# JuliaGeometry/Raycore.jl

Measured on AMD Instinct MI355X. Metric: Mrays/s closest_hit (1M-tri TLAS), higher is better.
Workload: dtype f32; 1 GPU; C3: TLAS of 256 rotated/scaled instances of one 4096-triangle BLAS (1 048 576 triangles), 4194304 pinhole primary rays per GPU per step, closest_hit; triangles=1048576, kernel=auto (phased persistent, top level in LDS), parallelism=replicas x1 (rays sharded, no collective)

## Files before the change

raycore.jl_amd/csrc/rc_build.hip:

```cpp
#include <hipcub/hipcub.hpp>
#include <rocprim/rocprim.hpp>

#include <algorithm>
#include <cmath>
#include <cstring>

#include "rc_internal.h"

namespace {

constexpr int kBlock = 256;
inline unsigned grid_for(uint64_t n) { return (unsigned)((n + kBlock - 1) / kBlock); }

__host__ __device__ inline uint32_t enc_f32(float f) {
    uint32_t u = __builtin_bit_cast(uint32_t, f);
    return (u & 0x80000000u) ? ~u : (u | 0x80000000u);
}
__host__ __device__ inline float dec_f32(uint32_t e) {
    uint32_t u = (e & 0x80000000u) ? (e & 0x7FFFFFFFu) : ~e;
    return __builtin_bit_cast(float, u);
}

__device__ inline void block_reduce_bounds(float3_ mn, float3_ mx, uint32_t* partials) {
    uint32_t e[6] = {enc_f32(mn.x), enc_f32(mn.y), enc_f32(mn.z), enc_f32(mx.x), enc_f32(mx.y), enc_f32(mx.z)};
// ... 744 lines not shown
    emit_tree(s, out.nodes.p, n, s->range_tmp);
    hipLaunchKernelGGL(k_blas_leaves, dim3(grid_for(n)), dim3(kBlock), 0, s->stream, out.nodes.p, out.prims.p, n);
    run_refit(s, out.nodes.p, out.prims.p, n, 0, s->range_tmp);
    rc_timing_scene_end(s, s->stream);
    RcNode root;
    RC_HIP(hipMemcpyAsync(&root, out.nodes.p, sizeof(RcNode), hipMemcpyDeviceToHost, s->stream));
    RC_HIP(hipStreamSynchronize(s->stream));
    RC_HIP(hipGetLastError());
    host_root_aabb(root, false, out.root_min, out.root_max);
}

static void pack_tlas(rc_scene* s) {
    const uint32_t n = (s->n_tlas_nodes + 1) / 2;
    if (s->tlas_top_k) hipLaunchKernelGGL(k_pack_nodes_remap, dim3(grid_for(s->n_tlas_nodes)), dim3(kBlock), 0, s->stream, s->tlas_nodes.p, s->flat_nodes.p + s->n_flat_nodes, s->n_tlas_nodes, n, s->tlas_remap.p, false);
    else hipLaunchKernelGGL(k_pack_nodes, dim3(grid_for(s->n_tlas_nodes)), dim3(kBlock), 0, s->stream, s->tlas_nodes.p, s->flat_nodes.p + s->n_flat_nodes, s->n_tlas_nodes, 0u);
}

void rc_build_tlas(rc_scene* s) {
    const uint32_t n = (uint32_t)s->instances.size();
    const uint32_t nb = (uint32_t)s->blas.size();
    s->descs.resize(nb);
    uint32_t tn = 0, tp = 0;
    for (uint32_t i = 0; i < nb; ++i) {
        s->descs[i].nodes_offset = tn; s->descs[i].primitives_offset = tp;
        memcpy(s->descs[i].root_min, s->blas[i].root_min, 12); memcpy(s->descs[i].root_max, s->blas[i].root_max, 12);
        tn += s->blas[i].n_nodes; tp += s->blas[i].n_prims;
    }
    s->n_flat_nodes = tn; s->n_flat_prims = tp;
    s->flat_attrs_valid = false;
    s->vf_order_valid = false;
    s->flat_nodes.reserve((size_t)tn + 2 * (size_t)n + 1);
    s->flat_prims.reserve(tp ? tp : 1);
    s->d_descs.reserve(nb ? nb : 1);
    s->blas_top_k = 0;
    s->tlas_top_k = 0;
    s->blas_top_k32 = 0;
    s->tlas_top_k32 = 0;
    s->small_trees = n <= rc::kStack16MaxLeaves;
    for (uint32_t i = 0; i < nb; ++i) s->small_trees = s->small_trees && s->blas[i].n_prims <= rc::kStack16MaxLeaves;
    const bool full_lds = n > 0 && 2 * n - 1 <= (uint32_t)rc::kTlasLdsNodes;
    const bool small_enough = (uint64_t)tn + 2ull * n < (1ull << 26);
    uint32_t blas_room = 0, blas_room32 = 0;
    auto split = [&](uint32_t P, uint32_t& tk, uint32_t& bk) {
        const uint32_t t_int = n - 1, b_int = (nb == 1 && s->blas[0].n_prims >= 2) ? s->blas[0].n_prims - 1 : 0;
        tk = t_int < P ? t_int : P; bk = b_int < P ? b_int : P;
        if (tk + bk > P) {
            const uint32_t half = P / 2;
            if (tk <= half) bk = P - tk; else if (bk <= half) tk = P - bk; else { tk = P - half; bk = half; }
        }
    };
    if (s->opt.blas_top && n > 0 && small_enough) {
        if (full_lds) {
            blas_room32 = (uint32_t)rc::kLdsPlaneNodes - (n - 1);
            blas_room = s->small_trees ? (uint32_t)rc::kLdsPlaneNodes16 - (n - 1) : blas_room32;
        } else {
            uint32_t tk, bk, tk32, bk32;
            split((uint32_t)rc::kPartialPlaneNodes, tk32, bk32);
            if (s->small_trees) split((uint32_t)rc::kPartialPlaneNodes16, tk, bk); else { tk = tk32; bk = bk32; }
            if (tk32 > tk) tk32 = tk;
            if (bk32 > bk) bk32 = bk;
            s->tlas_top_k = tk; s->tlas_top_k32 = tk32;
            blas_room = bk; blas_room32 = bk32;
        }
    }
    if (nb == 1 && blas_room > 0 && s->blas[0].n_prims >= 2) {
        const uint32_t n_leaves = s->blas[0].n_prims, n_int = n_leaves - 1, room = blas_room;
        s->blas_top_k = n_int < room ? n_int : room;
        s->blas_top_k32 = s->blas_top_k < blas_room32 ? s->blas_top_k : blas_room32;
        s->top_remap.reserve(n_int);
        hipLaunchKernelGGL(k_iota1, dim3(grid_for(n_int)), dim3(kBlock), 0, s->stream, s->top_remap.p, n_int);
        hipLaunchKernelGGL(k_top_remap, dim3(1), dim3(kTopBlock), 0, s->stream, s->blas[0].nodes.p, n_leaves, s->blas_top_k, s->top_remap.p);
    }
    for (uint32_t i = 0; i < nb; ++i) {
        if (s->blas_top_k) hipLaunchKernelGGL(k_pack_nodes_remap, dim3(grid_for(s->blas[i].n_nodes)), dim3(kBlock), 0, s->stream, s->blas[i].nodes.p, s->flat_nodes.p + s->descs[i].nodes_offset, s->blas[i].n_nodes, s->blas[i].n_prims, s->top_remap.p, true);
        else hipLaunchKernelGGL(k_pack_nodes, dim3(grid_for(s->blas[i].n_nodes)), dim3(kBlock), 0, s->stream, s->blas[i].nodes.p, s->flat_nodes.p + s->descs[i].nodes_offset, s->blas[i].n_nodes, s->blas[i].n_prims);
        RC_HIP(hipMemcpyAsync(s->flat_prims.p + s->descs[i].primitives_offset, s->blas[i].prims.p, sizeof(RcPrim) * s->blas[i].n_prims, hipMemcpyDeviceToDevice, s->stream));
    }
    if (nb) RC_HIP(hipMemcpyAsync(s->d_descs.p, s->descs.data(), sizeof(RcBlasDesc) * nb, hipMemcpyHostToDevice, s->stream));
    s->blas_nprims.resize(nb);
    for (uint32_t i = 0; i < nb; ++i) s->blas_nprims[i] = s->blas[i].n_prims;
    s->d_blas_nprims.reserve(nb ? nb : 1);
    if (nb) RC_HIP(hipMemcpyAsync(s->d_blas_nprims.p, s->blas_nprims.data(), sizeof(uint32_t) * nb, hipMemcpyHostToDevice, s->stream));
    s->blas_cull_bits.reserve(nb ? nb : 1);
    RC_HIP(hipMemsetAsync(s->blas_cull_bits.p, 0, sizeof(uint32_t) * (nb ? nb : 1), s->stream));
    if (nb && tp) hipLaunchKernelGGL(k_cull_radius, dim3(grid_for(tp)), dim3(kBlock), 0, s->stream, s->flat_prims.p, tp, s->d_descs.p, nb, s->blas_cull_bits.p);
    s->n_static_instances = n;
    if (n == 0) {
        s->n_tlas_nodes = 0;
        for (int k = 0; k < 3; ++k) { s->root_min[k] = INFINITY; s->root_max[k] = -INFINITY; }
        RC_HIP(hipStreamSynchronize(s->stream));
        return;
    }
    reserve_build_scratch(s, n);
    s->d_instances.reserve(n); s->inst_recs.reserve(n); s->inst_cull.reserve(2 * (size_t)n); s->aabb_tmp.reserve(6 * (size_t)n);
    s->tlas_nodes.reserve(2 * (size_t)n - 1);
    s->n_tlas_nodes = 2 * n - 1;
    RC_HIP(hipMemcpyAsync(s->d_instances.p, s->instances.data(), sizeof(RcInstanceDesc) * n, hipMemcpyHostToDevice, s->stream));
    hipLaunchKernelGGL(k_inst_recs, dim3(grid_for(n)), dim3(kBlock), 0, s->stream, s->d_instances.p, s->d_descs.p, s->d_blas_nprims.p, n, s->inst_recs.p,
                       (const uint32_t*)s->blas_cull_bits.p, s->inst_cull.p);
    s->bounds_partials.reserve((size_t)grid_for(n) * 6);
    hipLaunchKernelGGL(k_instance_aabbs, dim3(grid_for(n)), dim3(kBlock), 0, s->stream, s->d_instances.p, s->d_descs.p, n, s->aabb_tmp.p, s->bounds_partials.p);
    hipLaunchKernelGGL(k_reduce_partials, dim3(1), dim3(384), 0, s->stream, s->bounds_partials.p, grid_for(n), s->scene_enc.p);
    hipLaunchKernelGGL(k_tlas_morton, dim3(grid_for(n)), dim3(kBlock), 0, s->stream, s->d_instances.p, s->d_descs.p, n, s->scene_enc.p, s->keys_a.p, s->vals_a.p);
    sort_pairs(s, n);
    emit_tree(s, s->tlas_nodes.p, n, s->tlas_ranges);
    hipLaunchKernelGGL(k_tlas_leaves, dim3(grid_for(n)), dim3(kBlock), 0, s->stream, s->tlas_nodes.p, s->vals_b.p, s->d_instances.p, s->d_descs.p, n);
    run_refit(s, s->tlas_nodes.p, nullptr, n, 1, s->tlas_ranges);
// ... 35 lines not shown
```

raycore.jl_amd/csrc/rc_internal.h:

```cpp
#pragma once
#include <hip/hip_runtime.h>

#include <condition_variable>
#include <map>
#include <memory>
#include <mutex>
#include <set>
#include <stdexcept>
#include <string>
#include <vector>

#include "rc_device.h"

struct RcError : std::runtime_error {
    int code;
    RcError(int c, const std::string& m) : std::runtime_error(m), code(c) {}
};

#define RC_HIP(expr)                                                                                      \
    do {                                                                                                  \
        hipError_t _e = (expr);                                                                           \
        if (_e != hipSuccess)                                                                             \
            throw RcError(4, std::string(#expr) + " failed: " + hipGetErrorString(_e) + " (" __FILE__ ":" + \
                                 std::to_string(__LINE__) + ")");                                         \
// ... 37 lines not shown
    }
};

struct RcEvent {
    hipEvent_t e = nullptr;
    bool recorded = false, owned = false;
    RcEvent() = default;
    RcEvent(const RcEvent&) = delete;
    RcEvent& operator=(const RcEvent&) = delete;
    RcEvent(RcEvent&& o) noexcept : e(o.e), recorded(o.recorded), owned(o.owned) { o.e = nullptr; o.recorded = o.owned = false; }
    RcEvent& operator=(RcEvent&& o) noexcept { if (this != &o) { drop(); e = o.e; recorded = o.recorded; owned = o.owned; o.e = nullptr; o.recorded = o.owned = false; } return *this; }
    ~RcEvent() { drop(); }
    void drop() { if (e && owned) (void)hipEventDestroy(e); e = nullptr; recorded = owned = false; }
    void record(hipStream_t st) {
        if (e && !owned) drop();
        if (!e) { if (hipEventCreateWithFlags(&e, hipEventDisableTiming) != hipSuccess) { (void)hipGetLastError(); e = nullptr; return; } owned = true; }
        if (hipEventRecord(e, st) == hipSuccess) recorded = true; else (void)hipGetLastError();
    }
    void follow(hipEvent_t closing) { drop(); e = closing; recorded = closing != nullptr; }
    bool idle() const {
        if (!recorded) return true;
        const hipError_t q = hipEventQuery(e);
        if (q != hipSuccess) (void)hipGetLastError();
        return q == hipSuccess;
    }
    void wait() const { if (recorded && hipEventSynchronize(e) != hipSuccess) (void)hipGetLastError(); }
};

struct Blas {
    DevBuf<RcNode> nodes;
    DevBuf<RcPrim> prims;
    uint32_t n_prims = 0;
    uint32_t n_nodes = 0;
    float root_min[3] = {0, 0, 0}, root_max[3] = {0, 0, 0};
    DevBuf<float> m_normals, m_uvs;
    DevBuf<uint32_t> m_indices, src_face;
    bool has_attrs = false, has_uvs = false;
    uint32_t n_mesh_verts = 0, n_mesh_faces = 0;
    DevBuf<RcNode4> nodes4;
    uint32_t n_nodes4 = 0;
    uint32_t root_word4 = 1;
};

struct HandleRange {
    uint32_t first = 0, count = 0;
};

namespace rc {
constexpr int kTlasLdsNodes = 511;
constexpr int kTlasLdsInst = 256;
constexpr int kLdsPlaneNodes = 310;
constexpr int kPartialPlaneNodes = 585;
#ifndef RC_LDS_PLANES16
#define RC_LDS_PLANES16 748
#endif
constexpr int kLdsPlaneNodes16 = RC_LDS_PLANES16;
constexpr int kPartialPlaneNodes16 = 1023;
constexpr uint32_t kStack16MaxLeaves = 32767;
}

struct TraceOptions {
    int64_t kernel = -1;
    int64_t blocks_per_cu = 0;
    int64_t lds_stack = 24;
    int64_t pool = 0;
    int64_t refill = 20;
    int64_t sched_thr = 36;
    int64_t stats = 0;
    int64_t onesweep_min = 1000000;
    int64_t stack16 = 1;
    int64_t blas_top = 1;
    int64_t host_pipeline = 1;
    int64_t taper = 12;
    int64_t entry_cull = 1;
    int64_t cost_order = 1;
    int64_t cost_thr = 64;
    int64_t claim_shards = 16;
    int64_t vf_first_touch = 1;
    int64_t vf_chunk_bytes = 192 << 20;
    int64_t timeline_ptr = 0;
};

struct TimingRef {
    int slot = -2;
    uint64_t seq = 0;
    float fixed_ms = 0.f;
};

struct RcCaptureRelaxed {
    hipStreamCaptureMode mode = hipStreamCaptureModeRelaxed;
    RcCaptureRelaxed() { (void)hipThreadExchangeStreamCaptureMode(&mode); }
    ~RcCaptureRelaxed() { (void)hipThreadExchangeStreamCaptureMode(&mode); }
    RcCaptureRelaxed(const RcCaptureRelaxed&) = delete;
    RcCaptureRelaxed& operator=(const RcCaptureRelaxed&) = delete;
};

struct CallCtx {
    hipStream_t stream = nullptr;
    bool own_stream = false;
    bool busy = false;
    DevBuf<RcRay> rays;
    DevBuf<RcHit> hits;
};

struct rc_scene {
    int device = 0;
    int n_cus = 0;
    uint64_t uid = 0;
    hipStream_t stream = nullptr;
// ... 203 lines not shown
```

raycore.jl_amd/csrc/rc_traverse.hip:

```cpp
#include <algorithm>
#include <cstdlib>

#include <hip/hip_ext.h>
#include <hipcub/hipcub.hpp>

#include "rc_traverse_core.h"

namespace {

using namespace rc;

template <bool ANY, int LDS_N, int MINW>
__global__ __launch_bounds__(kBlock, MINW) void k_trace_simple(TraceArgs a) {
    __shared__ uint32_t lds_stack[LDS_N * kBlock];
    const uint32_t gtid = blockIdx.x * kBlock + threadIdx.x;
    LaneStackT<LDS_N> st(lds_stack + threadIdx.x, a.v.overflow + gtid, a.v.total_threads, a.v.status);
    for (uint64_t i = gtid; i < a.n_rays; i += a.v.total_threads) {
        RayState s;
        init_ray(s, load_ray(a.rays, i), ANY, st, a.v.tlas_off);
        if (a.v.n_tlas_nodes != 0)
            while (step<ANY>(s, a.v, st)) {}
        write_hit(s, a.v, a.hits, i);
    }
}
// ... 19 lines not shown
    s.node = RC_INVALID_NODE;
    unsigned long long st_steps = 0, st_lanes = 0, st_maxsp = 0;
    for (;;) {
        unsigned long long idle_mask = __ballot(!active);
        int n_idle = __popcll(idle_mask);
        const bool can_refill = !(exhausted && pool_next == pool_end);
        if (n_idle == 64 && !can_refill) break;
        if (can_refill && n_idle >= a.refill) {
            for (;;) {
                idle_mask = __ballot(!active);
                n_idle = __popcll(idle_mask);
                if (n_idle == 0) break;
                if (pool_next == pool_end) {
                    if (exhausted) break;
                    if (!rc_claim_chunk(a.claim, nullptr, (blockIdx.x * kBlock + threadIdx.x) >> 6, lane, a.n_rays, pool_next, pool_end)) { exhausted = true; break; }
                }
                const unsigned long long left = pool_end - pool_next;
                const unsigned rank = __builtin_amdgcn_mbcnt_hi((unsigned)(idle_mask >> 32),
                                                                __builtin_amdgcn_mbcnt_lo((unsigned)idle_mask, 0u));
                if (!active && rank < left) {
                    my_ray = pool_next + rank;
                    init_ray(s, load_ray(a.rays, my_ray), ANY, st, a.v.tlas_off);
                    active = true;
                }
                pool_next += ((unsigned long long)n_idle < left) ? (unsigned long long)n_idle : left;
            }
        }
        if (STATS) { st_steps += 1; st_lanes += active ? 1 : 0; if ((unsigned)s.sp > st_maxsp && active) st_maxsp = s.sp; }
        if (active) {
            if (!step<ANY>(s, a.v, st)) {
                write_hit(s, a.v, a.hits, my_ray);
                active = false;
            }
        }
    }
    if (STATS) {
        if (lane == 0) atomicAdd(&a.stats[0], st_steps);
        atomicAdd(&a.stats[1], st_lanes);
        atomicMax(&a.stats[2], st_maxsp);
    }
}

constexpr int kBigBlock = 1024;
constexpr size_t kBigStackBytes = (size_t)kLdsStack * kBigBlock * 4;
constexpr size_t kBigLdsBytes = kBigStackBytes + kLdsTopBytes;

template <bool ANY, int BLOCK, int LDS_N, int MINW, bool TIMELINE = false, bool STATS = false, bool STACK16 = false>
__global__ __launch_bounds__(BLOCK, MINW) void k_trace_phased_lds(TraceArgs a) {
    extern __shared__ __attribute__((aligned(16))) unsigned char smem[];
    typedef typename std::conditional<STACK16, uint16_t, uint32_t>::type entry_t;
    constexpr size_t stack_bytes = (size_t)LDS_N * BLOCK * sizeof(entry_t);
    constexpr int kPlanes = STACK16 ? kLdsPlaneNodes16 : kLdsPlaneNodes;
    entry_t* lds_stack = reinterpret_cast<entry_t*>(smem);
    const LdsTop top(smem + stack_bytes, (size_t)7 * kPlanes * sizeof(float2));
    if (a.v.n_tlas_nodes) stage_lds_top<BLOCK, kPlanes>(top, a.v, a.blas_k, a.lds_blas_base);
    __syncthreads();
    PersistArgs p{a.n_rays, a.claim, a.refill, a.sched_thr, a.stats, a.blas_k, a.lds_blas_base, 0u, a.timeline};
    phased_trace<ANY, LDS_N, STATS, ArraySource, HitWriter, BLOCK, true, true, false, TIMELINE, STACK16>(a.v, p, lds_stack, ArraySource{a.rays}, HitWriter{a.v.inst, a.hits}, top);
}

template <bool ANY, bool STACK16 = false>
__global__ __launch_bounds__(kMidBlock, 6) void k_trace_phased_partial(TraceArgs a) {
    extern __shared__ __attribute__((aligned(16))) unsigned char smem[];
    typedef typename std::conditional<STACK16, uint16_t, uint32_t>::type entry_t;
    entry_t* lds_stack = reinterpret_cast<entry_t*>(smem);
    LdsTop top;
    top.tl = reinterpret_cast<float2*>(smem + (size_t)kMidStack * kMidBlock * sizeof(entry_t));
    stage_partial_top<kMidBlock, STACK16 ? kPartialPlaneNodes16 : kPartialPlaneNodes>(top.tl, a.v, a.tlas_k, a.blas_k, a.lds_blas_base);
    __syncthreads();
    PersistArgs p{a.n_rays, a.claim, a.refill, a.sched_thr, a.stats, a.blas_k, a.lds_blas_base, a.tlas_k};
    phased_trace<ANY, kMidStack, false, ArraySource, HitWriter, kMidBlock, false, false, true, false, STACK16>(a.v, p, lds_stack, ArraySource{a.rays}, HitWriter{a.v.inst, a.hits}, top);
}

enum : int { K_EMPTY = 0, K_INTERIOR = 1, K_LEAF = 2, K_SWITCH = 3, K_DONE = 4 };

template <bool ANY, int LDS_N, int MINW, bool STATS>
__global__ __launch_bounds__(kBlock, MINW) void k_trace_sched(TraceArgs a) {
    __shared__ uint32_t lds_stack[LDS_N * kBlock];
    const uint32_t gtid = blockIdx.x * kBlock + threadIdx.x;
    LaneStackT<LDS_N> st(lds_stack + threadIdx.x, a.v.overflow + gtid, a.v.total_threads, a.v.status);
    const int lane = threadIdx.x & 63;
    if (a.v.n_tlas_nodes == 0) {
        RayState miss;
        miss.closest_inst = -1;
        for (uint64_t i = gtid; i < a.n_rays; i += a.v.total_threads) write_hit(miss, a.v, a.hits, i);
        return;
    }
    const uint32_t n_instances = (a.v.n_tlas_nodes + 1u) >> 1;
    const uint32_t tlas_off = a.v.tlas_off;
    const RcNode* const nodes = a.v.blas_nodes;
    unsigned long long pool_next = 0, pool_end = 0;
    bool exhausted = false;
    uint64_t my_ray = 0;
    float3_ wo = mk3(0, 0, 0), wd = mk3(0, 0, 0);
    float3_ o = mk3(0, 0, 0), d = mk3(0, 0, 0), inv = mk3(0, 0, 0), ox = mk3(0, 0, 0);
    float tmin = 0.f, closest_t = 0.f, hit_u = 0.f, hit_v = 0.f;
    uint32_t closest_prim = RC_INVALID_NODE, node = RC_INVALID_NODE, cur_off = 0, n_level = 0;
    int closest_inst = -1, cur_inst = -1, sp = 0, kind = K_EMPTY;
    unsigned long long st_iter[4] = {0, 0, 0, 0}, st_lane[4] = {0, 0, 0, 0};

    auto classify = [&](uint32_t nd) -> int {
        if (nd == RC_INVALID_NODE) return K_DONE;
        if (nd == RC_TOP_LEVEL_SENTINEL) return K_SWITCH;
        if (nd < n_level) return K_INTERIOR;
        return cur_inst < 0 ? K_SWITCH : K_LEAF;
    };

    for (;;) {
// ... 666 lines not shown
        h->next_record = h->gen + 7 + (h->records_asked % 3);
        h->records_asked += 1;
        if (h->rebuild_credit < 1) h->rebuild_credit = 1;
    }
    const float ex = s->root_max[0] - s->root_min[0], ey = s->root_max[1] - s->root_min[1], ez = s->root_max[2] - s->root_min[2];
    const float l2 = ex * ex + ey * ey + ez * ez;
    c.inv_l2 = (l2 > 0.f && l2 < 1e30f) ? 1.0f / l2 : 0.f;
    c.sample_rays = d_rays;
    c.n_sample = n;
    for (int k = 0; k < 8; ++k) c.sample_host[k] = host_sample ? host_sample[k] : 0.f;
    c.samples = h->samples.p;
    c.host_streak = h->fresh_streak.p;
    c.host_gen = (uint32_t)h->gen & 0xFFFFFFu;
    c.init_thr = (uint32_t)s->opt.cost_thr;
    c.order = h->order.p;
    c.cost = h->cost.p;
    c.hist = h->ctl.p;
    c.parity = h->parity;
    h->parity ^= 1u;
    return true;
}

void rc_launch_trace(rc_scene* s, const RcRay* d_rays, RcHit* d_hits, uint64_t n, int any_hit, hipStream_t stream, bool learn_order) {
    if (n == 0) return;
    RcLaunchGuard launch(s, stream);
    uint64_t want = (n + kBlock - 1) / kBlock, cap = (uint64_t)s->n_cus * rc_blocks_per_cu(s);
    uint32_t blocks = (uint32_t)(want < cap ? want : cap);
    uint32_t total_threads = blocks * kBlock;
    int64_t kernel = s->opt.kernel;
    if (kernel < 0)
        kernel = (n < (uint64_t)total_threads * 5 / 4) ? 0 : (s->n_tlas_nodes <= (uint32_t)kTlasLdsNodes ? 5 : 6);
    if (kernel == 4 && (s->n_tlas_nodes > (uint32_t)kTlasLdsNodes || s->n_static_instances > (uint32_t)kTlasLdsInst)) kernel = 3;
    if (kernel == 5 && s->n_tlas_nodes > (uint32_t)kTlasLdsNodes) kernel = 3;
    if (kernel == 6 && s->tlas_top_k + s->blas_top_k == 0) kernel = 3;
    if (kernel >= 3 && ((uint64_t)(s->n_flat_nodes + s->n_tlas_nodes) * 64u >= (1ull << 32) || n >= (1ull << 38))) kernel = 1;
    if (kernel == 4) {
        blocks = (uint32_t)std::min<uint64_t>((n + kBigBlock - 1) / kBigBlock, (uint64_t)s->n_cus);
        total_threads = blocks * kBigBlock;
    }
    if (kernel == 5 || kernel == 6) {
        blocks = (uint32_t)std::min<uint64_t>((n + kMidBlock - 1) / kMidBlock, (uint64_t)s->n_cus * (s->opt.blocks_per_cu == 1 ? 1 : 2));
        total_threads = blocks * kMidBlock;
    }
    TraceArgs a;
    a.v = rc_scene_view(s, total_threads);
    if (any_hit && s->opt.entry_cull < 2) a.v.inst_cull = nullptr;
    a.rays = d_rays; a.hits = d_hits; a.n_rays = n;
    rc_claim_fill(s, n, total_threads / 64u, a.claim);
    a.refill = (int)s->opt.refill;
    a.sched_thr = kernel == 2 ? 32 : (int)s->opt.sched_thr;
    a.stats = rc_stats_words(s);
    a.timeline = reinterpret_cast<unsigned long long*>(s->opt.timeline_ptr);
    const bool wide = rc_stack16(s);
    if ((kernel == 5 || kernel == 4) && s->opt.blas_top) { a.blas_k = (wide && kernel == 5) ? s->blas_top_k : s->blas_top_k32; a.lds_blas_base = (s->n_tlas_nodes + 1) / 2 - 1; }
    if (kernel == 6) {
        a.tlas_k = wide ? s->tlas_top_k : s->tlas_top_k32; a.blas_k = s->opt.blas_top ? (wide ? s->blas_top_k : s->blas_top_k32) : 0; a.lds_blas_base = a.tlas_k;
    }
    launch.bind();
    if (learn_order && (kernel == 3 || kernel == 5 || kernel == 6) && !launch.capturing) rc_cost_order_setup(s, n, any_hit, stream, a.claim, d_rays);
    if (any_hit) launch_variant<true>(s, kernel, a, blocks, stream); else launch_variant<false>(s, kernel, a, blocks, stream);
    launch.finish();
}
```

raycore.jl_amd/csrc/rc_traverse_core.h:

```cpp
#pragma once
#include <type_traits>

#include "rc_internal.h"

namespace rc {

constexpr int kBlock = 256;
constexpr int kLdsStack = 24;
constexpr int kTotalStack = 128;

struct SceneView {
    const RcNode* tlas_nodes;
    const RcNode* blas_nodes;
    const RcInstRec* inst;
    const RcPrim* prims;
    uint32_t n_tlas_nodes;
    uint32_t n_prims;
    uint32_t tlas_off;
    uint32_t n_nodes_total;
    uint32_t n_inst;
    const float4* inst_cull;
    uint32_t* overflow;
    uint32_t total_threads;
    uint32_t* status;
// ... 383 lines not shown
        const unsigned long long i = first + 2ull * (unsigned long long)lane;
        return i < end ? *reinterpret_cast<const uint32_t*>(rays + i) : 0u;
    }
};
struct HitWriter {
    const RcInstRec* inst;
    RcHit* hits;
    __device__ inline void operator()(uint64_t i, bool hit, float t, float u, float v, uint32_t prim, int instance) const {
        uint4 w0, w1;
        if (hit) {
            const uint4 m3 = *(reinterpret_cast<const uint4*>(inst + instance) + 3);
            w0 = make_uint4(1u, __float_as_uint(t), m3.y + prim - 1u, m3.z);
            w1 = make_uint4(__float_as_uint(u), __float_as_uint(v), (uint32_t)instance, 0u);
        } else {
            w0 = make_uint4(0u, 0u, RC_INVALID_NODE, 0u);
            w1 = make_uint4(0u, 0u, RC_INVALID_NODE, 0u);
        }
        uint4* out = reinterpret_cast<uint4*>(hits + i);
        out[0] = w0;
        out[1] = w1;
    }
};

typedef unsigned int u4v __attribute__((ext_vector_type(4)));
typedef unsigned int u2v __attribute__((ext_vector_type(2)));
__device__ inline __amdgpu_buffer_rsrc_t make_rsrc(const void* p, uint32_t bytes) {
    return __builtin_amdgcn_make_buffer_rsrc(const_cast<void*>(p), 0, bytes, 0x00020000);
}
__device__ inline float4 buf_f4(__amdgpu_buffer_rsrc_t r, uint32_t off, int soff = 0) {
    u4v v = __builtin_amdgcn_raw_buffer_load_b128(r, off, soff, 0);
    return make_float4(__uint_as_float(v.x), __uint_as_float(v.y), __uint_as_float(v.z), __uint_as_float(v.w));
}
__device__ inline float2 buf_f2(__amdgpu_buffer_rsrc_t r, uint32_t off, int soff = 0) {
    u2v v = __builtin_amdgcn_raw_buffer_load_b64(r, off, soff, 0);
    return make_float2(__uint_as_float(v.x), __uint_as_float(v.y));
}

struct PersistArgs {
    uint64_t n_items;
    RcClaim claim;
    int refill;
    int int_thr;
    unsigned long long* stats;
    uint32_t blas_k = 0;
    uint32_t lds_blas_base = 0;
    uint32_t tlas_k = 0;
    unsigned long long* timeline = nullptr;
};


constexpr int kMidBlock = 768, kMidStack = 16;
constexpr size_t kNodePlaneBytes = (size_t)7 * kLdsPlaneNodes * sizeof(float2);
constexpr size_t kLeafTableBytes = (size_t)kTlasLdsInst * sizeof(uint32_t);
constexpr size_t kInstPlaneBytes = (size_t)7 * kTlasLdsInst * sizeof(float2);
constexpr size_t kLdsTopBytes = kNodePlaneBytes + kLeafTableBytes + kInstPlaneBytes;
constexpr size_t kMidLdsBytes = (size_t)kMidStack * kMidBlock * 4 + kLdsTopBytes;
constexpr size_t kNodePlaneBytes16 = (size_t)7 * kLdsPlaneNodes16 * sizeof(float2);
constexpr size_t kMidLdsBytes16 = (size_t)kMidStack * kMidBlock * 2 + kNodePlaneBytes16 + kLeafTableBytes + kInstPlaneBytes;
#if RC_LDS_PLANES16 == 748
static_assert(kMidLdsBytes <= 81920 && kMidLdsBytes16 <= 81920, "two workgroups per CU share 160 KiB of LDS");
#else
static_assert(kMidLdsBytes <= 81920 && kMidLdsBytes16 <= 163840, "one workgroup per CU has 160 KiB of LDS");
#endif
struct LdsTop {
    float2* tl;
    uint32_t* lt;
    float2* il;
    __device__ inline explicit LdsTop(unsigned char* base, size_t node_plane_bytes = kNodePlaneBytes)
        : tl(reinterpret_cast<float2*>(base)), lt(reinterpret_cast<uint32_t*>(base + node_plane_bytes)),
          il(reinterpret_cast<float2*>(base + node_plane_bytes + kLeafTableBytes)) {}
    __device__ inline LdsTop() : tl(nullptr), lt(nullptr), il(nullptr) {}
};
template <int BLOCK, int PLANE_NODES = kLdsPlaneNodes>
__device__ inline void stage_lds_top(const LdsTop& t, const SceneView& v, uint32_t blas_k, uint32_t lds_blas_base) {
    const RcNode* tnodes = v.blas_nodes + v.tlas_off;
    const uint32_t n_inst = (v.n_tlas_nodes + 1u) >> 1;
    for (uint32_t i = threadIdx.x; i < (n_inst - 1u) * 7u; i += BLOCK) {
        const uint32_t nd = i / 7u, p = i % 7u;
        t.tl[p * PLANE_NODES + nd] = reinterpret_cast<const float2*>(tnodes + nd)[p];
    }
    for (uint32_t i = threadIdx.x; i < blas_k * 7u; i += BLOCK) {
        const uint32_t nd = i / 7u, p = i % 7u;
        t.tl[p * PLANE_NODES + lds_blas_base + nd] = reinterpret_cast<const float2*>(v.blas_nodes + nd)[p];
    }
    for (uint32_t j = threadIdx.x; j < n_inst; j += BLOCK)
        t.lt[j] = reinterpret_cast<const uint32_t*>(tnodes + (n_inst - 1u + j))[13];
    for (uint32_t i = threadIdx.x; i < v.n_inst * 7u; i += BLOCK) {
        const uint32_t in = i / 7u, p = i % 7u;
        const uint32_t* rec = reinterpret_cast<const uint32_t*>(v.inst + in);
        const uint32_t a = p < 6u ? rec[2u * p] : rec[12], b = p < 6u ? rec[2u * p + 1u] : rec[15];
        t.il[p * kTlasLdsInst + in] = make_float2(__uint_as_float(a), __uint_as_float(b));
    }
}

constexpr size_t kPartialPlaneBytes = (size_t)7 * kPartialPlaneNodes * sizeof(float2);
constexpr size_t kPartialLdsBytes = (size_t)kMidStack * kMidBlock * 4 + kPartialPlaneBytes;
constexpr size_t kPartialPlaneBytes16 = (size_t)7 * kPartialPlaneNodes16 * sizeof(float2);
constexpr size_t kPartialLdsBytes16 = (size_t)kMidStack * kMidBlock * 2 + kPartialPlaneBytes16;
static_assert(kPartialLdsBytes <= 81920 && kPartialLdsBytes16 <= 81920, "two workgroups per CU share 160 KiB of LDS");
template <int BLOCK, int PLANE_NODES = kPartialPlaneNodes>
__device__ inline void stage_partial_top(float2* tl, const SceneView& v, uint32_t tlas_k, uint32_t blas_k, uint32_t lds_blas_base) {
    const RcNode* tnodes = v.blas_nodes + v.tlas_off;
    for (uint32_t i = threadIdx.x; i < tlas_k * 7u; i += BLOCK) {
        const uint32_t nd = i / 7u, p = i % 7u;
        tl[p * PLANE_NODES + nd] = reinterpret_cast<const float2*>(tnodes + nd)[p];
    }
    for (uint32_t i = threadIdx.x; i < blas_k * 7u; i += BLOCK) {
        const uint32_t nd = i / 7u, p = i % 7u;
        tl[p * PLANE_NODES + lds_blas_base + nd] = reinterpret_cast<const float2*>(v.blas_nodes + nd)[p];
    }
}

__device__ inline float rcp_rn_normal(float d) {
    float r = __builtin_amdgcn_rcpf(d);
    const float e = __builtin_fmaf(-d, r, 1.0f);
    r = __builtin_fmaf(e, r, r);
    float q = r;
    const float e2 = __builtin_fmaf(-d, q, 1.0f);
    q = __builtin_fmaf(e2, r, q);
    const float e3 = __builtin_fmaf(-d, q, 1.0f);
    return __builtin_fmaf(e3, r, q);
}
__device__ inline float3_ safe_inv3(const float3_ d) {
    const float ooeps = 1.0e-5f;
    const float ax = __builtin_fabsf(d.x), ay = __builtin_fabsf(d.y), az = __builtin_fabsf(d.z);
    const bool tame = __builtin_fmaxf(__builtin_fmaxf(ax, ay), az) < 0x1p60f && ax == ax && ay == ay && az == az;
    if (__builtin_expect(__ballot(!tame) == 0ull, 1)) {
        const float cx = ax > ooeps ? d.x : __builtin_copysignf(ooeps, d.x), cy = ay > ooeps ? d.y : __builtin_copysignf(ooeps, d.y),
                    cz = az > ooeps ? d.z : __builtin_copysignf(ooeps, d.z);
        return mk3(rcp_rn_normal(cx), rcp_rn_normal(cy), rcp_rn_normal(cz));
    }
    return mk3(safe_inv1(d.x), safe_inv1(d.y), safe_inv1(d.z));
}

#ifdef RC_PHASE_MARKERS
#define RC_MARK(name) asm volatile("; RC_MARK " name)
#else
#define RC_MARK(name) ((void)0)
#endif

template <bool ANY, int LDS_N, bool STATS, class Source, class Sink, int BLOCK = kBlock, bool TLAS_LDS = false, bool INST_LDS = TLAS_LDS, bool PARTIAL_LDS = false,
          bool TIMELINE = false, bool STACK16 = false>
__device__ inline void phased_trace(const SceneView& av, const PersistArgs& a, typename std::conditional<STACK16, uint16_t, uint32_t>::type* lds_stack, const Source& src,
                                    const Sink& sink, const LdsTop top = LdsTop()) {
    typedef typename std::conditional<STACK16, uint16_t, uint32_t>::type stack_entry_t;
    constexpr uint32_t kInv = STACK16 ? 0xFFFFu : RC_INVALID_NODE, kSent = STACK16 ? 0xFFFEu : RC_TOP_LEVEL_SENTINEL;
    const float2* const tl = top.tl;
    const uint32_t* const lt = top.lt;
    const float2* const il = top.il;
    const uint32_t gtid = blockIdx.x * BLOCK + threadIdx.x;
    LaneStackP<LDS_N, BLOCK, stack_entry_t> st(lds_stack + threadIdx.x, av.overflow + gtid, av.total_threads, av.status);
    const int lane = threadIdx.x & 63;
    if (av.n_tlas_nodes == 0) {
        for (uint64_t i = gtid; i < a.n_items; i += av.total_threads) sink(i, false, 0.0f, 0.0f, 0.0f, RC_INVALID_NODE, -1);
        return;
    }
    const uint32_t n_instances = (av.n_tlas_nodes + 1u) >> 1;
    const uint32_t tlas_off = av.tlas_off;
    const __amdgpu_buffer_rsrc_t nrs1 = make_rsrc(reinterpret_cast<const char*>(av.blas_nodes) - 64, (av.n_nodes_total + 1u) * 64u);
    const __amdgpu_buffer_rsrc_t irs = make_rsrc(av.inst, av.n_inst * 64u);
    const bool cull_on = av.inst_cull != nullptr;
    const __amdgpu_buffer_rsrc_t crs = make_rsrc(av.inst_cull, cull_on ? av.n_inst * 32u : 0u);
    float c_idd = 0.f, c_idl = 0.f, c_ray = 0.f, c_dd = 0.f;
    unsigned long long pool_next = 0, pool_end = 0;
    bool exhausted = false;
    uint64_t my_ray = 0;
    float3_ wo = mk3(0, 0, 0), wd = mk3(0, 0, 0), winv = mk3(0, 0, 0);
    float3_ inv = mk3(0, 0, 0), ox = mk3(0, 0, 0);
    v2f oyz = {0.f, 0.f}, ozx = {0.f, 0.f}, dyz = {0.f, 0.f}, dzx = {0.f, 0.f};
    float tmin = 0.f, closest_t = 0.f, hit_u = 0.f, hit_v = 0.f;
    uint32_t closest_prim = RC_INVALID_NODE, cur_off = 0, n_level = 0;
    uint32_t node = kInv;
    int closest_inst = -1, cur_inst = -1;
    uint32_t it_total = 0, start_it = 0;
    const uint32_t* claim_order = a.claim.order;
    uint32_t* claim_cost = a.claim.cost;
    uint32_t life_thr = 0xFFFFFFFFu;
    if (a.claim.hist) {
        float smp[8];
        const OrderDecision od = order_select(a.claim, lane, smp);
        const uint32_t sel = od.sel;
        claim_order = __builtin_amdgcn_readfirstlane(od.valid) ? claim_order + (size_t)sel * kHistSlotStride : nullptr;
        life_thr = __builtin_amdgcn_readfirstlane(od.life_thr);
        claim_cost = life_thr == 0xFFFFFFFFu ? nullptr : claim_cost + (size_t)sel * kHistSlotStride;
        if (__builtin_amdgcn_readfirstlane(od.fresh) && !__builtin_amdgcn_readfirstlane(od.paused)) {
            uint32_t* stale = a.claim.cost + (size_t)sel * kHistSlotStride;
            const uint64_t n_base = (a.n_items + a.claim.pool - 1u) / a.claim.pool;
            for (uint64_t i = gtid; i < n_base; i += av.total_threads) stale[i] = 0u;
        }
        if (blockIdx.x == 0 && threadIdx.x < 64) order_commit(a.claim, od, lane, smp);
    }
    typename LaneStackP<LDS_N, BLOCK, stack_entry_t>::pos_t sp = st.empty();
    bool live = false;
    unsigned long long st_iter[4] = {0, 0, 0, 0}, st_lane[4] = {0, 0, 0, 0}, st_outer = 0, st_sub[4] = {0, 0, 0, 0}, st_cull = 0;
    unsigned long long st_t0 = STATS ? wall_clock64() : 0ull, st_tx = 0ull;
    int thr_eff = __builtin_amdgcn_readfirstlane(a.int_thr);
    unsigned long long tl_t0 = TIMELINE ? wall_clock64() : 0ull, tl_tx = 0ull, tl_t16 = 0ull, tl_t4 = 0ull;
    uint32_t tl_outer = 0, tl_outer_x = 0, tl_live_x = 0, tl_int = 0, tl_int_x = 0;

    for (;;) {
#if defined(RC_AGE_PRIO)
        {
// ... 50 lines not shown
                if (far_ok) st.push(sp, far_c);
                node = near_ok ? near_c : st.pop(sp);
            }
            RC_MARK("interior_end");
            if (n_int < thr_eff) break;
        }
        {
            const bool is_leaf = cur_inst >= 0 && node >= n_level && node < kSent;
            if (STATS && __ballot(is_leaf)) { st_iter[2] += 1; st_lane[2] += is_leaf ? 1 : 0; }
            RC_MARK("leaf_begin");
            if (is_leaf) {
                const uint32_t off = (cur_off + node) << 6;
                const float4 qa = buf_f4(nrs1, off), qb = buf_f4(nrs1, off, 16), qc = buf_f4(nrs1, off, 32);
                const v2f A0 = {qa.x, qa.y}, A1 = {qa.z, qa.w}, B0 = {qb.x, qb.y}, B1 = {qb.z, qb.w}, C0 = {qc.x, qc.y}, C1 = {qc.z, qc.w};
                const float e1x = B0.y, e1y = B1.x, e1z = B0.x, e2x = C0.y, e2y = C1.x, e2z = C0.x, dx = dzx.y, dy = dyz.x, dz = dyz.y;
                const v2f s1xy = dyz * C0 - dzx * C1;
                const float s1z = dx * e2y - dy * e2x;
                const float det = (s1xy.x * e1x + s1xy.y * e1y) + s1z * e1z;
                const float invd = 1.0f / det;
                const v2f ddyz = oyz - A0, ddzx = ozx - A1;
                const float ddx = ddzx.y, ddy = ddyz.x, ddz = ddyz.y;
                const float u = ((ddx * s1xy.x + ddy * s1xy.y) + ddz * s1z) * invd;
                const v2f s2xy = ddyz * B0 - ddzx * B1;
                const float s2z = ddx * e1y - ddy * e1x;
                const float v = ((dx * s2xy.x + dy * s2xy.y) + dz * s2z) * invd;
                const float t = ((e2x * s2xy.x + e2y * s2xy.y) + e2z * s2z) * invd;
                const bool hit = !(u < 0.0f || u > 1.0f) && !(v < 0.0f || (u + v) > 1.0f) && !(t < tmin || t > closest_t);
                closest_prim = hit ? node - n_level + 1u : closest_prim;
                closest_inst = hit ? cur_inst : closest_inst;
                closest_t = hit ? t : closest_t;
                hit_u = hit ? u : hit_u;
                hit_v = hit ? v : hit_v;
                if (ANY && hit) node = kInv;
                else node = st.pop(sp);
            }
            RC_MARK("leaf_end");
        }
        bool was_skipped = false;
        {
            const bool is_exit = node == kSent;
            const bool is_entry = cur_inst < 0 && node >= n_level && node < kSent;
            if (STATS && __ballot(is_exit || is_entry)) { st_iter[3] += 1; st_lane[3] += (is_exit || is_entry) ? 1 : 0; }
            if (STATS) { if (__ballot(is_exit)) st_sub[0] += 1; if (__ballot(is_entry)) st_sub[1] += 1; }
            RC_MARK("switch_begin");
            if (is_exit) {
                node = st.pop(sp);
                cur_inst = -1;
                cur_off = tlas_off; n_level = n_instances;
                inv = winv;
                ox = mk3(-wo.x * inv.x, -wo.y * inv.y, -wo.z * inv.z);
                RC_MARK("switch_end");
            } else if (is_entry) {
                RC_MARK("entry_begin");
                float4 m0, m1, m2;
                u4v m3;
                if (TLAS_LDS) cur_inst = (int)lt[node - n_level];
                else cur_inst = (int)__builtin_amdgcn_raw_buffer_load_b32(nrs1, (cur_off + node) << 6, 52, 0);
                bool skip = false;
                if (cull_on) {
                    const float4 cs = buf_f4(crs, (uint32_t)cur_inst << 5);
                    const float cB = __uint_as_float(__builtin_amdgcn_raw_buffer_load_b32(crs, (uint32_t)cur_inst << 5, 16, 0));
                    const float Lx = cs.x - wo.x, Ly = cs.y - wo.y, Lz = cs.z - wo.z;
                    const float LL = __builtin_fmaf(Lz, Lz, __builtin_fmaf(Ly, Ly, Lx * Lx));
                    const float bq = __builtin_fmaf(Lz, wd.z, __builtin_fmaf(Ly, wd.y, Lx * wd.x));
                    const float tc = bq * c_idd;
                    const float d2 = __builtin_fmaf(-4.0e-6f, LL, __builtin_fmaf(-tc, bq, LL));
                    const float ts = __builtin_amdgcn_fmed3f(tc, tmin, closest_t) - tc;
                    const float seg = __builtin_fmaf(0.999f * ts * ts, c_dd, d2);
                    const float Ae = cs.w + c_ray;
                    const float tb = 2.0f * __builtin_fmaf(Ae, c_idl, __builtin_fabsf(tc));
                    const float R = __builtin_fmaf(__builtin_fmaf(5.0e-6f, c_dd * c_idl, cB), tb, Ae);
                    skip = seg > R * R;
                }
                if (STATS) was_skipped = skip;
                if (skip) {
                    cur_inst = -1;
                    node = st.pop(sp);
                } else {
                if (INST_LDS) {
                    const float2* q = il + cur_inst;
                    const float2 p0 = q[0], p1 = q[kTlasLdsInst], p2 = q[2 * kTlasLdsInst], p3 = q[3 * kTlasLdsInst],
                                 p4 = q[4 * kTlasLdsInst], p5 = q[5 * kTlasLdsInst], p6 = q[6 * kTlasLdsInst];
                    m0 = make_float4(p0.x, p0.y, p1.x, p1.y); m1 = make_float4(p2.x, p2.y, p3.x, p3.y); m2 = make_float4(p4.x, p4.y, p5.x, p5.y);
                    m3 = u4v{__float_as_uint(p6.x), 0u, 0u, __float_as_uint(p6.y)};
                } else {
                    const uint32_t ioff = (uint32_t)cur_inst << 6;
                    m0 = buf_f4(irs, ioff); m1 = buf_f4(irs, ioff, 16); m2 = buf_f4(irs, ioff, 32);
                    m3 = __builtin_amdgcn_raw_buffer_load_b128(irs, ioff, 48, 0);
                }
                st.push(sp, kSent);
                node = 1;
                cur_off = m3.x;
                n_level = m3.w;
                const float3_ o = mk3(m0.x * wo.x + m0.y * wo.y + m0.z * wo.z + m0.w, m1.x * wo.x + m1.y * wo.y + m1.z * wo.z + m1.w,
                                      m2.x * wo.x + m2.y * wo.y + m2.z * wo.z + m2.w);
                const float3_ d = mk3(m0.x * wd.x + m0.y * wd.y + m0.z * wd.z, m1.x * wd.x + m1.y * wd.y + m1.z * wd.z,
                                      m2.x * wd.x + m2.y * wd.y + m2.z * wd.z);
                oyz = v2f{o.y, o.z}; ozx = v2f{o.z, o.x}; dyz = v2f{d.y, d.z}; dzx = v2f{d.z, d.x};
                inv = safe_inv3(d);
                ox = mk3(-o.x * inv.x, -o.y * inv.y, -o.z * inv.z);
                }
                RC_MARK("entry_end");
            }
        }
        if (STATS) st_cull += (unsigned long long)__popcll(__ballot(was_skipped));
        {
            RC_MARK("finish_begin");
            if (STATS) st_outer += 1;
            const bool fin = live && node == kInv;
            const int n_free = __popcll(__ballot(fin || !live));
            const bool can_refill = !(exhausted && pool_next == pool_end);
            if (STATS && !can_refill && st_tx == 0) st_tx = wall_clock64();
            if (TIMELINE) {
                tl_outer += 1;
                if (!can_refill) {
                    const uint32_t n_live = 64u - (uint32_t)n_free;
                    if (tl_tx == 0) tl_tx = wall_clock64();
                    tl_outer_x += 1; tl_live_x += n_live;
                    if (n_live < 16u && tl_t16 == 0) tl_t16 = wall_clock64();
                    if (n_live < 4u && tl_t4 == 0) tl_t4 = wall_clock64();
                }
            }
            if (!can_refill) {
                const int half_live = (64 - n_free) / 2;
                thr_eff = __builtin_amdgcn_readfirstlane(half_live < a.int_thr ? (half_live > 1 ? half_live : 1) : a.int_thr);
            }
            if (n_free == 64 && !can_refill && !__ballot(fin)) break;
            if (n_free >= a.refill || n_free == 64 || !can_refill) {
                if (STATS && __ballot(fin)) st_sub[2] += 1;
                RC_MARK("finish_end");
                RC_MARK("writeout_begin");
                if (fin) {
                    sink(my_ray, closest_inst >= 0, closest_t, hit_u, hit_v, closest_prim, closest_inst);
                    live = false;
                    const uint32_t life = it_total - start_it;
                    if (claim_cost && life >= life_thr) atomicMax(claim_cost + (uint32_t)(my_ray >> a.claim.pool_shift), life);
                }
                RC_MARK("writeout_end");
// ... 96 lines not shown
```

Before: 7751 Mrays/s.

## Stage per-slot instance cull spheres in LDS and index instance planes by leaf slot

Instance transform planes are now stored under the TLAS leaf slot index rather than the instance id. For the 16-bit-stack path, a new LDS region holds each instance's cull sphere and its instance id, so the entry step reads everything from LDS instead of issuing dependent global buffer loads for the leaf instance id and the cull data. To fit the extra planes, the 16-bit BLAS node-plane capacity is reduced from 748 to 658 nodes and blas_k is clamped to match. This trades fewer BLAS top nodes resident in LDS for cheaper instance entry, and the LDS budget static_assert is switched to the two-workgroups-per-CU case for the new size.

```diff
diff --git a/raycore.jl_amd/csrc/rc_build.hip b/raycore.jl_amd/csrc/rc_build.hip
--- a/raycore.jl_amd/csrc/rc_build.hip
+++ b/raycore.jl_amd/csrc/rc_build.hip
@@ -820,7 +820,7 @@
     if (s->opt.blas_top && n > 0 && small_enough) {
         if (full_lds) {
             blas_room32 = (uint32_t)rc::kLdsPlaneNodes - (n - 1);
-            blas_room = s->small_trees ? (uint32_t)rc::kLdsPlaneNodes16 - (n - 1) : blas_room32;
+            blas_room = s->small_trees ? (uint32_t)rc::kTopOrderNodes16 - (n - 1) : blas_room32;
         } else {
             uint32_t tk, bk, tk32, bk32;
             split((uint32_t)rc::kPartialPlaneNodes, tk32, bk32);
diff --git a/raycore.jl_amd/csrc/rc_internal.h b/raycore.jl_amd/csrc/rc_internal.h
--- a/raycore.jl_amd/csrc/rc_internal.h
+++ b/raycore.jl_amd/csrc/rc_internal.h
@@ -113,9 +113,10 @@
 constexpr int kLdsPlaneNodes = 310;
 constexpr int kPartialPlaneNodes = 585;
 #ifndef RC_LDS_PLANES16
-#define RC_LDS_PLANES16 748
+#define RC_LDS_PLANES16 658
 #endif
 constexpr int kLdsPlaneNodes16 = RC_LDS_PLANES16;
+constexpr int kTopOrderNodes16 = kLdsPlaneNodes16 > 748 ? kLdsPlaneNodes16 : 748;
 constexpr int kPartialPlaneNodes16 = 1023;
 constexpr uint32_t kStack16MaxLeaves = 32767;
 }
diff --git a/raycore.jl_amd/csrc/rc_traverse.hip b/raycore.jl_amd/csrc/rc_traverse.hip
--- a/raycore.jl_amd/csrc/rc_traverse.hip
+++ b/raycore.jl_amd/csrc/rc_traverse.hip
@@ -95,8 +95,8 @@
     constexpr size_t stack_bytes = (size_t)LDS_N * BLOCK * sizeof(entry_t);
     constexpr int kPlanes = STACK16 ? kLdsPlaneNodes16 : kLdsPlaneNodes;
     entry_t* lds_stack = reinterpret_cast<entry_t*>(smem);
-    const LdsTop top(smem + stack_bytes, (size_t)7 * kPlanes * sizeof(float2));
-    if (a.v.n_tlas_nodes) stage_lds_top<BLOCK, kPlanes>(top, a.v, a.blas_k, a.lds_blas_base);
+    const LdsTop top(smem + stack_bytes, (size_t)7 * kPlanes * sizeof(float2), STACK16);
+    if (a.v.n_tlas_nodes) stage_lds_top<BLOCK, kPlanes, STACK16>(top, a.v, a.blas_k, a.lds_blas_base);
     __syncthreads();
     PersistArgs p{a.n_rays, a.claim, a.refill, a.sched_thr, a.stats, a.blas_k, a.lds_blas_base, 0u, a.timeline};
     phased_trace<ANY, LDS_N, STATS, ArraySource, HitWriter, BLOCK, true, true, false, TIMELINE, STACK16>(a.v, p, lds_stack, ArraySource{a.rays}, HitWriter{a.v.inst, a.hits}, top);
@@ -869,7 +869,10 @@
     a.stats = rc_stats_words(s);
     a.timeline = reinterpret_cast<unsigned long long*>(s->opt.timeline_ptr);
     const bool wide = rc_stack16(s);
-    if ((kernel == 5 || kernel == 4) && s->opt.blas_top) { a.blas_k = (wide && kernel == 5) ? s->blas_top_k : s->blas_top_k32; a.lds_blas_base = (s->n_tlas_nodes + 1) / 2 - 1; }
+    if ((kernel == 5 || kernel == 4) && s->opt.blas_top) {
+        a.lds_blas_base = (s->n_tlas_nodes + 1) / 2 - 1;
+        a.blas_k = (wide && kernel == 5) ? std::min(s->blas_top_k, (uint32_t)kLdsPlaneNodes16 - a.lds_blas_base) : s->blas_top_k32;
+    }
     if (kernel == 6) {
         a.tlas_k = wide ? s->tlas_top_k : s->tlas_top_k32; a.blas_k = s->opt.blas_top ? (wide ? s->blas_top_k : s->blas_top_k32) : 0; a.lds_blas_base = a.tlas_k;
     }
diff --git a/raycore.jl_amd/csrc/rc_traverse_core.h b/raycore.jl_amd/csrc/rc_traverse_core.h
--- a/raycore.jl_amd/csrc/rc_traverse_core.h
+++ b/raycore.jl_amd/csrc/rc_traverse_core.h
@@ -459,26 +459,30 @@
 constexpr int kMidBlock = 768, kMidStack = 16;
 constexpr size_t kNodePlaneBytes = (size_t)7 * kLdsPlaneNodes * sizeof(float2);
 constexpr size_t kLeafTableBytes = (size_t)kTlasLdsInst * sizeof(uint32_t);
+constexpr size_t kEntryPlaneBytes = (size_t)3 * kTlasLdsInst * sizeof(float2);
 constexpr size_t kInstPlaneBytes = (size_t)7 * kTlasLdsInst * sizeof(float2);
 constexpr size_t kLdsTopBytes = kNodePlaneBytes + kLeafTableBytes + kInstPlaneBytes;
 constexpr size_t kMidLdsBytes = (size_t)kMidStack * kMidBlock * 4 + kLdsTopBytes;
 constexpr size_t kNodePlaneBytes16 = (size_t)7 * kLdsPlaneNodes16 * sizeof(float2);
-constexpr size_t kMidLdsBytes16 = (size_t)kMidStack * kMidBlock * 2 + kNodePlaneBytes16 + kLeafTableBytes + kInstPlaneBytes;
-#if RC_LDS_PLANES16 == 748
+constexpr size_t kMidLdsBytes16 = (size_t)kMidStack * kMidBlock * 2 + kNodePlaneBytes16 + kEntryPlaneBytes + kInstPlaneBytes;
+#if RC_LDS_PLANES16 == 658
 static_assert(kMidLdsBytes <= 81920 && kMidLdsBytes16 <= 81920, "two workgroups per CU share 160 KiB of LDS");
 #else
 static_assert(kMidLdsBytes <= 81920 && kMidLdsBytes16 <= 163840, "one workgroup per CU has 160 KiB of LDS");
 #endif
+static_assert(kLdsPlaneNodes >= kTlasLdsInst - 1 && kLdsPlaneNodes16 >= kTlasLdsInst - 1, "the node planes hold every TLAS interior node");
 struct LdsTop {
     float2* tl;
     uint32_t* lt;
+    float2* ec;
     float2* il;
-    __device__ inline explicit LdsTop(unsigned char* base, size_t node_plane_bytes = kNodePlaneBytes)
-        : tl(reinterpret_cast<float2*>(base)), lt(reinterpret_cast<uint32_t*>(base + node_plane_bytes)),
-          il(reinterpret_cast<float2*>(base + node_plane_bytes + kLeafTableBytes)) {}
-    __device__ inline LdsTop() : tl(nullptr), lt(nullptr), il(nullptr) {}
-};
-template <int BLOCK, int PLANE_NODES = kLdsPlaneNodes>
+    __device__ inline explicit LdsTop(unsigned char* base, size_t node_plane_bytes = kNodePlaneBytes, bool entry_planes = false)
+        : tl(reinterpret_cast<float2*>(base)), lt(entry_planes ? nullptr : reinterpret_cast<uint32_t*>(base + node_plane_bytes)),
+          ec(entry_planes ? reinterpret_cast<float2*>(base + node_plane_bytes) : nullptr),
+          il(reinterpret_cast<float2*>(base + node_plane_bytes + (entry_planes ? kEntryPlaneBytes : kLeafTableBytes))) {}
+    __device__ inline LdsTop() : tl(nullptr), lt(nullptr), ec(nullptr), il(nullptr) {}
+};
+template <int BLOCK, int PLANE_NODES = kLdsPlaneNodes, bool ENTRY_PLANES = false>
 __device__ inline void stage_lds_top(const LdsTop& t, const SceneView& v, uint32_t blas_k, uint32_t lds_blas_base) {
     const RcNode* tnodes = v.blas_nodes + v.tlas_off;
     const uint32_t n_inst = (v.n_tlas_nodes + 1u) >> 1;
@@ -490,13 +494,21 @@
         const uint32_t nd = i / 7u, p = i % 7u;
         t.tl[p * PLANE_NODES + lds_blas_base + nd] = reinterpret_cast<const float2*>(v.blas_nodes + nd)[p];
     }
-    for (uint32_t j = threadIdx.x; j < n_inst; j += BLOCK)
-        t.lt[j] = reinterpret_cast<const uint32_t*>(tnodes + (n_inst - 1u + j))[13];
-    for (uint32_t i = threadIdx.x; i < v.n_inst * 7u; i += BLOCK) {
-        const uint32_t in = i / 7u, p = i % 7u;
-        const uint32_t* rec = reinterpret_cast<const uint32_t*>(v.inst + in);
-        const uint32_t a = p < 6u ? rec[2u * p] : rec[12], b = p < 6u ? rec[2u * p + 1u] : rec[15];
-        t.il[p * kTlasLdsInst + in] = make_float2(__uint_as_float(a), __uint_as_float(b));
+    constexpr uint32_t kSlotPlanes = ENTRY_PLANES ? 10u : 8u;
+    for (uint32_t i = threadIdx.x; i < n_inst * kSlotPlanes; i += BLOCK) {
+        const uint32_t j = i / kSlotPlanes, p = i % kSlotPlanes;
+        const uint32_t in = reinterpret_cast<const uint32_t*>(tnodes + (n_inst - 1u + j))[13];
+        if (p < 7u) {
+            const uint32_t* rec = reinterpret_cast<const uint32_t*>(v.inst + in);
+            const uint32_t a = p < 6u ? rec[2u * p] : rec[12], b = p < 6u ? rec[2u * p + 1u] : rec[15];
+            t.il[p * kTlasLdsInst + j] = make_float2(__uint_as_float(a), __uint_as_float(b));
+        } else if (!ENTRY_PLANES) {
+            t.lt[j] = in;
+        } else {
+            const float4 c = v.inst_cull ? v.inst_cull[2u * in] : make_float4(0.f, 0.f, 0.f, 0.f);
+            const float cB = v.inst_cull ? v.inst_cull[2u * in + 1u].x : 0.f;
+            t.ec[(p - 7u) * kTlasLdsInst + j] = p == 7u ? make_float2(c.x, c.y) : p == 8u ? make_float2(c.z, c.w) : make_float2(cB, __uint_as_float(in));
+        }
     }
 }
 
@@ -540,6 +552,21 @@
     return mk3(safe_inv1(d.x), safe_inv1(d.y), safe_inv1(d.z));
 }
 
+__device__ inline bool entry_culled(const float4 cs, const float cB, const float3_ wo, const float3_ wd, const float c_idd, const float c_idl,
+                                    const float c_ray, const float c_dd, const float tmin, const float closest_t) {
+    const float Lx = cs.x - wo.x, Ly = cs.y - wo.y, Lz = cs.z - wo.z;
+    const float LL = __builtin_fmaf(Lz, Lz, __builtin_fmaf(Ly, Ly, Lx * Lx));
+    const float bq = __builtin_fmaf(Lz, wd.z, __builtin_fmaf(Ly, wd.y, Lx * wd.x));
+    const float tc = bq * c_idd;
+    const float d2 = __builtin_fmaf(-4.0e-6f, LL, __builtin_fmaf(-tc, bq, LL));
+    const float ts = __builtin_amdgcn_fmed3f(tc, tmin, closest_t) - tc;
+    const float seg = __builtin_fmaf(0.999f * ts * ts, c_dd, d2);
+    const float Ae = cs.w + c_ray;
+    const float tb = 2.0f * __builtin_fmaf(Ae, c_idl, __builtin_fabsf(tc));
+    const float R = __builtin_fmaf(__builtin_fmaf(5.0e-6f, c_dd * c_idl, cB), tb, Ae);
+    return seg > R * R;
+}
+
 #ifdef RC_PHASE_MARKERS
 #define RC_MARK(name) asm volatile("; RC_MARK " name)
 #else
@@ -554,7 +581,10 @@
     constexpr uint32_t kInv = STACK16 ? 0xFFFFu : RC_INVALID_NODE, kSent = STACK16 ? 0xFFFEu : RC_TOP_LEVEL_SENTINEL;
     const float2* const tl = top.tl;
     const uint32_t* const lt = top.lt;
+    const float2* const ec = top.ec;
     const float2* const il = top.il;
+    static_assert(TLAS_LDS == INST_LDS, "LdsTop keeps a TLAS leaf's instance index and the instance's record under the same slot index");
+    constexpr bool ENTRY_LDS = INST_LDS && STACK16;
     const uint32_t gtid = blockIdx.x * BLOCK + threadIdx.x;
     LaneStackP<LDS_N, BLOCK, stack_entry_t> st(lds_stack + threadIdx.x, av.overflow + gtid, av.total_threads, av.status);
     const int lane = threadIdx.x & 63;
@@ -711,38 +741,47 @@
                 RC_MARK("switch_end");
             } else if (is_entry) {
                 RC_MARK("entry_begin");
+#if defined(RC_EXP_ENTRY_NOP)
+#pragma unroll
+                for (int k = 0; k < RC_EXP_ENTRY_NOP; ++k) asm volatile("s_nop 15");
+#endif
                 float4 m0, m1, m2;
                 u4v m3;
-                if (TLAS_LDS) cur_inst = (int)lt[node - n_level];
-                else cur_inst = (int)__builtin_amdgcn_raw_buffer_load_b32(nrs1, (cur_off + node) << 6, 52, 0);
                 bool skip = false;
-                if (cull_on) {
-                    const float4 cs = buf_f4(crs, (uint32_t)cur_inst << 5);
-                    const float cB = __uint_as_float(__builtin_amdgcn_raw_buffer_load_b32(crs, (uint32_t)cur_inst << 5, 16, 0));
-                    const float Lx = cs.x - wo.x, Ly = cs.y - wo.y, Lz = cs.z - wo.z;
-                    const float LL = __builtin_fmaf(Lz, Lz, __builtin_fmaf(Ly, Ly, Lx * Lx));
-                    const float bq = __builtin_fmaf(Lz, wd.z, __builtin_fmaf(Ly, wd.y, Lx * wd.x));
-                    const float tc = bq * c_idd;
-                    const float d2 = __builtin_fmaf(-4.0e-6f, LL, __builtin_fmaf(-tc, bq, LL));
-                    const float ts = __builtin_amdgcn_fmed3f(tc, tmin, closest_t) - tc;
-                    const float seg = __builtin_fmaf(0.999f * ts * ts, c_dd, d2);
-                    const float Ae = cs.w + c_ray;
-                    const float tb = 2.0f * __builtin_fmaf(Ae, c_idl, __builtin_fabsf(tc));
-                    const float R = __builtin_fmaf(__builtin_fmaf(5.0e-6f, c_dd * c_idl, cB), tb, Ae);
-                    skip = seg > R * R;
+                if (ENTRY_LDS) {
+                    const uint32_t j = node - n_level;
+                    const float2 e2 = ec[2 * kTlasLdsInst + j];
+                    const float2* q = il + j;
+                    const float2 p0 = q[0], p1 = q[kTlasLdsInst], p2 = q[2 * kTlasLdsInst], p3 = q[3 * kTlasLdsInst],
+                                 p4 = q[4 * kTlasLdsInst], p5 = q[5 * kTlasLdsInst], p6 = q[6 * kTlasLdsInst];
+                    m0 = make_float4(p0.x, p0.y, p1.x, p1.y); m1 = make_float4(p2.x, p2.y, p3.x, p3.y); m2 = make_float4(p4.x, p4.y, p5.x, p5.y);
+                    m3 = u4v{__float_as_uint(p6.x), 0u, 0u, __float_as_uint(p6.y)};
+                    cur_inst = (int)__float_as_uint(e2.y);
+                    if (cull_on) {
+                        const float2 e0 = ec[j], e1 = ec[kTlasLdsInst + j];
+                        skip = entry_culled(make_float4(e0.x, e0.y, e1.x, e1.y), e2.x, wo, wd, c_idd, c_idl, c_ray, c_dd, tmin, closest_t);
+                    }
+                } else {
+                    if (TLAS_LDS) cur_inst = (int)lt[node - n_level];
+                    else cur_inst = (int)__builtin_amdgcn_raw_buffer_load_b32(nrs1, (cur_off + node) << 6, 52, 0);
+                    if (cull_on) {
+                        const float4 cs = buf_f4(crs, (uint32_t)cur_inst << 5);
+                        const float cB = __uint_as_float(__builtin_amdgcn_raw_buffer_load_b32(crs, (uint32_t)cur_inst << 5, 16, 0));
+                        skip = entry_culled(cs, cB, wo, wd, c_idd, c_idl, c_ray, c_dd, tmin, closest_t);
+                    }
                 }
                 if (STATS) was_skipped = skip;
                 if (skip) {
                     cur_inst = -1;
                     node = st.pop(sp);
                 } else {
-                if (INST_LDS) {
-                    const float2* q = il + cur_inst;
+                if (INST_LDS && !ENTRY_LDS) {
+                    const float2* q = il + (node - n_level);
                     const float2 p0 = q[0], p1 = q[kTlasLdsInst], p2 = q[2 * kTlasLdsInst], p3 = q[3 * kTlasLdsInst],
                                  p4 = q[4 * kTlasLdsInst], p5 = q[5 * kTlasLdsInst], p6 = q[6 * kTlasLdsInst];
                     m0 = make_float4(p0.x, p0.y, p1.x, p1.y); m1 = make_float4(p2.x, p2.y, p3.x, p3.y); m2 = make_float4(p4.x, p4.y, p5.x, p5.y);
                     m3 = u4v{__float_as_uint(p6.x), 0u, 0u, __float_as_uint(p6.y)};
-                } else {
+                } else if (!INST_LDS) {
                     const uint32_t ioff = (uint32_t)cur_inst << 6;
                     m0 = buf_f4(irs, ioff); m1 = buf_f4(irs, ioff, 16); m2 = buf_f4(irs, ioff, 32);
                     m3 = __builtin_amdgcn_raw_buffer_load_b128(irs, ioff, 48, 0);
```

Result: no change. 7819 Mrays/s, median of 6 (+0.9%).
